# faasm/faabric

Measured on AMD Instinct MI355X. Metric: MPI_Allreduce GB/s + batch-exec msgs/sec, 8-rank world at 1/2/4/8 MI355X, higher is better.
Workload: dtype fp32; 1 GPU; model=faabric composite: 256MB fp32 allreduce + 1MB alltoall + kvtouch batch, global_batch=128, parallelism=mpi1, allreduce_bytes=268435456, pingpong_bytes=0, kv_bytes=4096, full=False, snapshot_bytes_per_rank=0, snapshot_dirty=random-scattered 25pct, random-byte region, gpu=True

## Files before the change

### cpp/bindings/bindings_runtime.cpp

```cpp
#include <pybind11/functional.h>
#include <pybind11/pybind11.h>
#include <pybind11/stl.h>

#include "faabricamd/endpoint.h"
#include "faabricamd/executor.h"
#include "faabricamd/flat.h"
#include "faabricamd/hipipc.h"
#include "faabricamd/mpi.h"
#include "faabricamd/planner.h"
#include "faabricamd/ptp.h"
#include "faabricamd/runner.h"
#include "faabricamd/scheduler.h"
#include "faabricamd/snapshot.h"
#include "faabricamd/state.h"
#include "faabricamd/util.h"
#include "faabricamd/utilextras.h"
#include "faabricamd/dirty.h"
#include <hip/hip_runtime.h>

namespace py = pybind11;
using namespace faabricamd;

namespace faabricamd {
void registerBenchFunctions();
// ... 767 lines not shown
    m.def("prof_summary", &profSummary);
    m.def("prof_clear", &profClear);
    m.def("set_up_crash_handler", &setUpCrashHandler);
    m.def("pin_thread_to_free_cpu", &pinThreadToFreeCpu);

    m.def("_selftest_segfault_tracker", [] {
        py::gil_scoped_release release;
        SegfaultDirtyTracker tracker;
        PageAlignedBuffer buf;
        buf.resize(16 * 4096);
        tracker.startTracking(buf.data(), buf.size());
        buf.data()[3 * 4096 + 5] = 42;
        buf.data()[9 * 4096] = 7;
        tracker.stopTracking(buf.data(), buf.size());
        auto dirty = tracker.getDirtyPages(buf.data(), buf.size());
        int nDirty = 0;
        for (char c : dirty) {
            nDirty += c != 0;
        }
        return nDirty == 2 && dirty[3] == 1 && dirty[9] == 1;
    });

    m.def("_selftest_uffd_tracker", []() -> py::object {
        if (!UffdDirtyTracker::isAvailable()) {
            return py::none();
        }
        bool ok;
        {
            py::gil_scoped_release release;
            UffdDirtyTracker tracker;
            PageAlignedBuffer buf;
            buf.resize(16 * 4096);
            tracker.startTracking(buf.data(), buf.size());
            buf.data()[2 * 4096 + 11] = 42;
            buf.data()[14 * 4096] = 7;
            tracker.stopTracking(buf.data(), buf.size());
            auto dirty = tracker.getDirtyPages(buf.data(), buf.size());
            int nDirty = 0;
            for (char d : dirty) {
                nDirty += d != 0;
            }
            ok = nDirty == 2 && dirty[2] == 1 && dirty[14] == 1;
        }
        return py::bool_(ok);
    });

    m.def("_selftest_softpte_tracker", []() -> py::object {
        if (!SoftPTEDirtyTracker::isAvailable()) {
            return py::none();
        }
        bool ok;
        {
            py::gil_scoped_release release;
            SoftPTEDirtyTracker tracker;
            PageAlignedBuffer buf;
            buf.resize(16 * 4096);
            std::memset(buf.data(), 1, buf.size());
            tracker.startTracking(buf.data(), buf.size());
            buf.data()[5 * 4096 + 3] = 42;
            buf.data()[12 * 4096] = 7;
            tracker.stopTracking(buf.data(), buf.size());
            auto dirty = tracker.getDirtyPages(buf.data(), buf.size());
            ok = dirty.size() == 16 && dirty[5] == 1 && dirty[12] == 1;
        }
        return py::bool_(ok);
    });

    m.def("_debug_runtime_sizes", [] {
        py::dict d;
        d["planner_app_results"] = Planner::get().debugAppResultsCount();
        d["planner_done_apps"] = Planner::get().debugDoneAppsCount();
        d["planner_in_flight"] = Planner::get().debugInFlightCount();
        d["broker_mappings"] = getPointToPointBroker().debugMappingsCount();
        d["broker_channels"] = getPointToPointBroker().debugChannelsCount();
        d["broker_send_seqs"] = getPointToPointBroker().debugSendSeqsCount();
        d["decision_cache"] = DecisionCache::get().size();
        return d;
    });
    m.def("_debug_dispatch_sizes", [] {
        py::dict d;
        d["idle_executors"] = Scheduler::get().debugIdleCount();
        d["planner_msg_index_apps"] = Planner::get().debugMsgIndexCount();
        d["planner_used_slots"] = Planner::get().debugUsedSlots();
        return d;
    });
    m.def("_debug_current_executor_id", [] {
        return ExecutorContext::get().getExecutor()->id;
    });
    m.def("_debug_set_message_result", [](const Message& msg) {
        auto copy = std::make_shared<Message>(msg);
        py::gil_scoped_release release;
        getPlannerClient().setMessageResult(copy);
    });
    m.def("_debug_kv_commit_stats", [] {
        KvCommitStats s = kvCommitStats();
        py::dict d;
        d["launches"] = s.launches;
        d["pages"] = s.pages;
        return d;
    });
    m.def("_debug_kv_sweep_bitmap",
          [](size_t nPages, const std::vector<uint64_t>& setBits) {
              size_t nWords = (nPages + 63) / 64;
              auto words = std::make_unique<std::atomic<uint64_t>[]>(
                std::max<size_t>(nWords, 1));
              for (size_t w = 0; w < nWords; w++) {
                  words[w].store(0);
              }
              for (uint64_t b : setBits) {
                  if (b >= nPages) {
                      throw FaabricException("bit beyond the bitmap");
                  }
                  words[b / 64].fetch_or(1ULL << (b % 64));
              }
              std::vector<uint32_t> pages(nPages);
              size_t n =
                kvSweepDirtyBitmap(words.get(), nPages, pages.data());
              pages.resize(n);
              std::vector<uint64_t> after(nWords);
              for (size_t w = 0; w < nWords; w++) {
                  after[w] = words[w].load();
              }
              return py::make_tuple(pages, after);
          },
          py::arg("n_pages"),
          py::arg("set_bits"));
    m.def("_debug_op_reduce_host",
          [](int op, int dtype, const py::bytes& inBytes,
             const py::bytes& inoutBytes) {
              if (op < 0 || op > (int)MpiOp::PROD || dtype < 0 ||
                  dtype > (int)MpiDataType::BYTE) {
                  throw FaabricException("bad op or dtype");
              }
              std::string in = inBytes;
              std::string inout = inoutBytes;
              size_t elem = mpiTypeSize((MpiDataType)dtype);
              if (in.size() != inout.size() || (in.size() % elem) != 0) {
                  throw FaabricException("operand length mismatch");
              }
              MpiWorld::opReduceHost((MpiOp)op,
                                     (MpiDataType)dtype,
                                     (int)(inout.size() / elem),
                                     (const uint8_t*)in.data(),
                                     (uint8_t*)inout.data());
              return py::bytes(inout.data(), inout.size());
          },
          py::arg("op"),
          py::arg("dtype"),
          py::arg("in_bytes"),
          py::arg("inout_bytes"));
    m.def("wait_batch_done",
          [](int32_t appId, int timeoutMs) {
              py::gil_scoped_release release;
              return getPlannerClient().waitBatchDone(appId, timeoutMs);
          },
          py::arg("app_id"),
          py::arg("timeout_ms") = 30000);
    m.def("set_bound_timeout",
          [](int ms) { getSystemConfig().boundTimeout = ms; });
    m.def("reap_stale_executors", [] {
        py::gil_scoped_release release;
        return Scheduler::get().reapStaleExecutors();
    });
    m.def("register_bench_functions", [] { registerBenchFunctions(); });
    m.def("bench_last_outputs", [] {
        py::dict d;
        for (const auto& [name, data] : benchLastOutputs()) {
            d[py::str(name)] =
// ... 167 lines not shown
```

### cpp/include/faabricamd/executor.h

```cpp
#pragma once

#include <atomic>
#include <functional>
#include <memory>
#include <string>
#include <thread>
#include <vector>

#include "faabricamd/mailbox.h"
#include "faabricamd/messages.h"
#include "faabricamd/queue.h"
#include "faabricamd/dirty.h"
#include "faabricamd/snapshot.h"

namespace faabricamd {

class Executor;


class ExecutorContext
{
  public:
    static bool isSet();
    static void set(Executor* executor,
                    std::shared_ptr<BatchExecuteRequest> req,
                    int msgIdx);
    static void unset();
    static ExecutorContext& get();

    Executor* getExecutor() const { return executor; }
    std::shared_ptr<BatchExecuteRequest> getBatchRequest() const
    {
        return req;
    }
    Message& getMsg();
    int getMsgIdx() const { return msgIdx; }

  private:
    Executor* executor = nullptr;
    std::shared_ptr<BatchExecuteRequest> req;
    int msgIdx = 0;
};


using FaabricFunction = std::function<int32_t(Message&)>;

class FunctionRegistry
{
  public:
    static FunctionRegistry& get();
    void registerFunction(const std::string& user,
                          const std::string& function,
                          FaabricFunction fn);
    FaabricFunction* getFunction(const std::string& user,
                                 const std::string& function);
    void clear();

  private:
    std::mutex mx;
    std::map<std::string, FaabricFunction> functions;
};


struct ExecutorTask
{
    ExecutorTask() = default;
    ExecutorTask(int msgIdxIn, std::shared_ptr<BatchExecuteRequest> reqIn)
      : msgIdx(msgIdxIn)
      , req(std::move(reqIn))
    {}
    int msgIdx = 0;
    std::shared_ptr<BatchExecuteRequest> req;
    bool stop = false;
    bool single = false;
    int64_t enqueueNs = 0;
};

class Executor : public std::enable_shared_from_this<Executor>
{
  public:
    explicit Executor(Message& msg);
    virtual ~Executor();

    void executeTasks(const std::vector<int>& msgIdxs,
                      const std::shared_ptr<BatchExecuteRequest>& req);
    void executeSingleTask(int msgIdx,
                           const std::shared_ptr<BatchExecuteRequest>& req);

    std::vector<std::pair<int32_t, int32_t>> executeThreads(
      std::shared_ptr<BatchExecuteRequest> req,
      const std::vector<SnapshotMergeRegion>& mergeRegions);

    virtual int32_t executeTask(int threadPoolIdx,
                                int msgIdx,
                                std::shared_ptr<BatchExecuteRequest> req);

    virtual std::pair<uint8_t*, size_t> getMemoryView();
    virtual void setMemorySize(size_t newSize);
    void setDeviceMemorySize(size_t newSize);
    std::pair<uint8_t*, size_t> getDeviceMemoryView();
    bool hasDeviceArena() const { return deviceArena != nullptr; }
    virtual void restore(const std::string& snapshotKey);
    virtual void reset(Message& msg);
    virtual void flush();

    bool tryClaim();
    void claim();
    void releaseClaim();
    bool isClaimed() const { return claimed.load(); }
    using IdleExecutors = IdleList<std::shared_ptr<Executor>>;
    void setIdleList(std::shared_ptr<IdleExecutors> list)
    {
        idleList = std::move(list);
    }

    long getMillisSinceLastExec() const;
    void shutdown();

    std::string id;
    Message boundMsg;
    int gpuDevice = -1;

    void setThreadResult(Message& msg,
                         int32_t returnValue,
                         const std::string& key,
                         const std::vector<SnapshotDiffMsg>& diffs);

  protected:
    void threadPoolThread(int poolIdx);
    void handleTaskResult(Message& msg,
                          int32_t returnValue,
                          std::shared_ptr<BatchExecuteRequest> req,
                          bool isLastInBatch);

    int threadPoolSize = 0;
    using TaskMailbox = Mailbox<ExecutorTask>;
    std::vector<std::unique_ptr<TaskMailbox>> threadMailboxes;
    std::vector<std::thread> threadPoolThreads;
    std::unique_ptr<std::atomic<bool>[]> poolThreadUp;
    std::mutex threadsMx;
    void ensurePoolThreadLocked(int poolIdx);
    void postTask(int poolIdx, ExecutorTask&& task);

    std::shared_ptr<IdleExecutors> idleList;

    std::atomic<bool> claimed{ false };
    std::atomic<int64_t> lastExecMs{ 0 };

    std::string lastForkSnapshotKey;
    std::vector<std::string> lastForkRemoteHosts;
    void cleanupForkSnapshot();

    std::shared_ptr<std::atomic<int>> batchCounter;

    PageAlignedBuffer dummyMemory;

    uint8_t* deviceArena = nullptr;
    size_t deviceArenaSize = 0;
};

class ExecutorFactory
{
  public:
    virtual ~ExecutorFactory() = default;
    virtual std::shared_ptr<Executor> createExecutor(Message& msg)
    {
        return std::make_shared<Executor>(msg);
    }
    virtual void flushHost() {}
};

void setExecutorFactory(std::shared_ptr<ExecutorFactory> factory);
std::shared_ptr<ExecutorFactory> getExecutorFactory();

int32_t chainFunction(const std::string& user,
                      const std::string& function,
                      const std::vector<uint8_t>& input);
Message awaitChainedCall(int32_t msgId, int timeoutMs = 60000);

int32_t migrationPoint(const std::vector<uint8_t>& reentryInput);

}
```

### cpp/include/faabricamd/mailbox.h

```cpp
#pragma once

#include <atomic>
#include <climits>
#include <cstddef>
#include <cstdint>
#include <ctime>
#include <mutex>
#include <utility>
#include <vector>

#include <linux/futex.h>
#include <sys/syscall.h>
#include <unistd.h>

namespace faabricamd {

namespace detail {

inline void futexWait(std::atomic<uint32_t>* word,
                      uint32_t expected,
                      int timeoutMs)
{
    static_assert(sizeof(std::atomic<uint32_t>) == sizeof(uint32_t));
    struct timespec ts;
    struct timespec* tsp = nullptr;
    if (timeoutMs > 0) {
        ts.tv_sec = timeoutMs / 1000;
        ts.tv_nsec = (long)(timeoutMs % 1000) * 1000000L;
        tsp = &ts;
    }
    syscall(SYS_futex,
            reinterpret_cast<uint32_t*>(word),
            FUTEX_WAIT_PRIVATE,
            expected,
            tsp,
            nullptr,
            0);
}

inline void futexWake(std::atomic<uint32_t>* word, int n)
{
    syscall(SYS_futex,
            reinterpret_cast<uint32_t*>(word),
            FUTEX_WAKE_PRIVATE,
            n,
            nullptr,
            nullptr,
            0);
}

}

template<typename T, uint32_t SLOTS = 8>
class Mailbox
{
    static_assert(SLOTS >= 2 && (SLOTS & (SLOTS - 1)) == 0,
                  "SLOTS must be a power of two");

  public:
    Mailbox()
    {
        for (uint32_t i = 0; i < SLOTS; i++) {
            slots[i].seq.store(i, std::memory_order_relaxed);
        }
    }
    Mailbox(const Mailbox&) = delete;
    Mailbox& operator=(const Mailbox&) = delete;

    void post(T value)
    {
        uint32_t ticket = tail.fetch_add(1, std::memory_order_relaxed);
        Slot& s = slots[ticket & (SLOTS - 1)];
        uint32_t seen;
        while ((seen = s.seq.load(std::memory_order_acquire)) != ticket) {
            detail::futexWait(&s.seq, seen, 1);
        }
        s.value = std::move(value);
        s.seq.store(ticket + 1, std::memory_order_seq_cst);
        if (sleeping.load(std::memory_order_seq_cst) != 0) {
            detail::futexWake(&s.seq, INT_MAX);
        }
    }

    bool take(T& out, int timeoutMs)
    {
        Slot& s = slots[head & (SLOTS - 1)];
        uint32_t ready = head + 1;
        uint32_t seen = s.seq.load(std::memory_order_acquire);
        if (seen != ready) {
            struct timespec start;
            clock_gettime(CLOCK_MONOTONIC, &start);
            int leftMs = timeoutMs;
            while (true) {
                sleeping.store(1, std::memory_order_seq_cst);
                seen = s.seq.load(std::memory_order_seq_cst);
                if (seen != ready) {
                    detail::futexWait(&s.seq, seen, leftMs);
                    seen = s.seq.load(std::memory_order_acquire);
                }
                sleeping.store(0, std::memory_order_relaxed);
                if (seen == ready) {
                    break;
                }
                if (timeoutMs > 0) {
                    struct timespec now;
                    clock_gettime(CLOCK_MONOTONIC, &now);
                    int64_t goneMs =
                      (int64_t)(now.tv_sec - start.tv_sec) * 1000 +
                      (now.tv_nsec - start.tv_nsec) / 1000000;
                    if (goneMs >= timeoutMs) {
                        return false;
                    }
                    leftMs = (int)(timeoutMs - goneMs);
                }
            }
        }
        out = std::move(s.value);
        s.value = T();
        s.seq.store(head + SLOTS, std::memory_order_release);
        head++;
        return true;
    }

  private:
    struct alignas(64) Slot
    {
        std::atomic<uint32_t> seq{ 0 };
        T value{};
    };
    Slot slots[SLOTS];
    alignas(64) std::atomic<uint32_t> tail{ 0 };
    std::atomic<uint32_t> sleeping{ 0 };
    alignas(64) uint32_t head = 0;
};

template<typename T>
class IdleList
{
  public:
    void push(T value)
    {
        std::lock_guard<std::mutex> lock(mx);
        if (!closed) {
            entries.push_back(std::move(value));
        }
    }

    size_t popMany(size_t n, std::vector<T>& out)
    {
        std::lock_guard<std::mutex> lock(mx);
        size_t got = 0;
        while (got < n && !entries.empty()) {
            out.push_back(std::move(entries.back()));
            entries.pop_back();
            got++;
        }
        return got;
    }

    bool pop(T& out)
    {
        std::lock_guard<std::mutex> lock(mx);
        if (entries.empty()) {
            return false;
        }
        out = std::move(entries.back());
        entries.pop_back();
        return true;
    }

    size_t remove(const T& value)
    {
        std::lock_guard<std::mutex> lock(mx);
        size_t before = entries.size();
        size_t w = 0;
        for (size_t r = 0; r < entries.size(); r++) {
            if (!(entries[r] == value)) {
                if (w != r) {
                    entries[w] = std::move(entries[r]);
                }
                w++;
            }
        }
        entries.resize(w);
        return before - w;
    }

    void close()
    {
        std::vector<T> dropped;
        {
            std::lock_guard<std::mutex> lock(mx);
            closed = true;
            dropped.swap(entries);
        }
    }

    size_t size()
    {
        std::lock_guard<std::mutex> lock(mx);
        return entries.size();
    }

  private:
    std::mutex mx;
    std::vector<T> entries;
    bool closed = false;
};

}
```

### cpp/include/faabricamd/util.h

```cpp
#pragma once

#include <atomic>
#include <cstdarg>
#include <cstdint>
#include <cstring>
#include <string>
#include <vector>

namespace faabricamd {


enum class LogLevel : int
{
    trace = 0,
    debug = 1,
    info = 2,
    warn = 3,
    error = 4,
    off = 5,
};

LogLevel getLogLevel();
void setLogLevel(LogLevel lvl);
void logMessage(LogLevel lvl, const char* fmt, ...)
  __attribute__((format(printf, 2, 3)));

#define FAM_TRACE(...)                                                         \
    ::faabricamd::logMessage(::faabricamd::LogLevel::trace, __VA_ARGS__)
#define FAM_DEBUG(...)                                                         \
    ::faabricamd::logMessage(::faabricamd::LogLevel::debug, __VA_ARGS__)
#define FAM_INFO(...)                                                          \
    ::faabricamd::logMessage(::faabricamd::LogLevel::info, __VA_ARGS__)
#define FAM_WARN(...)                                                          \
    ::faabricamd::logMessage(::faabricamd::LogLevel::warn, __VA_ARGS__)
#define FAM_ERROR(...)                                                         \
    ::faabricamd::logMessage(::faabricamd::LogLevel::error, __VA_ARGS__)


class FaabricException : public std::exception
{
  public:
    explicit FaabricException(std::string msgIn)
      : msg(std::move(msgIn))
    {}
    const char* what() const noexcept override { return msg.c_str(); }

  private:
    std::string msg;
};

class FunctionMigratedException : public FaabricException
{
  public:
    using FaabricException::FaabricException;
};
class FunctionFrozenException : public FaabricException
{
  public:
    using FaabricException::FaabricException;
};

inline constexpr int MIGRATED_FUNCTION_RETURN_VALUE = -99;
inline constexpr int FROZEN_FUNCTION_RETURN_VALUE = -98;


std::string getEnvVar(const std::string& key, const std::string& deflt);
int getEnvVarInt(const std::string& key, int deflt);

int getUsableCores();

struct SystemConfig
{
    std::string logLevel;
    std::string endpointHost;
    std::string plannerHost;
    int plannerPort = 8011;

    std::string batchSchedulerMode;
    int overrideCpuCount = 0;
    int overrideGpuCount = -1;
    int gpuDevice = 0;
    bool gpuDevicePinned = false;
    bool useGpu = true;

    int globalMessageTimeout = 60000;
    int boundTimeout = 30000;

    int functionServerThreads = 4;
    int stateServerThreads = 2;
    int snapshotServerThreads = 2;
    int pointToPointServerThreads = 4;
    int plannerServerThreads = 4;

    std::string dirtyTrackingMode;
    std::string diffingMode;

    std::string stateMode;

    int defaultMpiWorldSize = 5;
    int mpiBasePort = 8020;

    void initialise();
    void print() const;
};

SystemConfig& getSystemConfig();


uint32_t generateGid();
int32_t generateGidInt32();


int64_t getGlobalClockEpochMillis();
int64_t getEpochMicros();
double getSecondsSinceEpoch();


bool startsWith(const std::string& value, const std::string& prefix);
bool endsWith(const std::string& value, const std::string& suffix);
std::string randomString(size_t len);

inline std::vector<uint8_t> stringToBytes(const std::string& s)
{
    return { s.begin(), s.end() };
}
inline std::string bytesToString(const std::vector<uint8_t>& b)
{
    return { b.begin(), b.end() };
}

template<typename T>
void appendBytesOf(std::vector<uint8_t>& out, const T& v)
{
    const auto* p = reinterpret_cast<const uint8_t*>(&v);
    out.insert(out.end(), p, p + sizeof(T));
}

template<typename T>
T readBytesAt(const uint8_t* data, size_t offset)
{
    T v;
    std::memcpy(&v, data + offset, sizeof(T));
    return v;
}


std::string getPrimaryIPForThisHost(const std::string& interface = "");


void setMockMode(bool value);
bool isMockMode();
void setTestMode(bool value);
bool isTestMode();


std::string funcToString(const std::string& user,
                         const std::string& function,
                         int messageId);

std::string getMainThreadSnapshotKey(const std::string& user,
                                     const std::string& function,
                                     int appId);

}
```

### cpp/src/executor.cpp

```cpp
#include "faabricamd/executor.h"
#include "faabricamd/utilextras.h"
#include "faabricamd/mpi.h"
#include "faabricamd/ops.h"
#include "faabricamd/planner.h"

#include <hip/hip_runtime.h>
#include "faabricamd/snapshot.h"
#include "faabricamd/util.h"

#include <algorithm>
#include <cstring>

namespace faabricamd {

void resultBatcherEnqueue(std::shared_ptr<Message> msg);


static thread_local std::shared_ptr<ExecutorContext> currentContext;

bool ExecutorContext::isSet()
{
    return currentContext != nullptr;
}

void ExecutorContext::set(Executor* executor,
                          std::shared_ptr<BatchExecuteRequest> req,
                          int msgIdx)
{
    auto ctx = std::make_shared<ExecutorContext>();
    ctx->executor = executor;
    ctx->req = std::move(req);
    ctx->msgIdx = msgIdx;
    currentContext = ctx;
}

void ExecutorContext::unset()
{
    currentContext = nullptr;
}

ExecutorContext& ExecutorContext::get()
{
    if (!currentContext) {
        throw FaabricException("no executor context set");
    }
    return *currentContext;
}

Message& ExecutorContext::getMsg()
{
    return req->messages.at(msgIdx);
}


FunctionRegistry& FunctionRegistry::get()
{
    static FunctionRegistry reg;
    return reg;
}

void FunctionRegistry::registerFunction(const std::string& user,
                                        const std::string& function,
                                        FaabricFunction fn)
{
    std::lock_guard<std::mutex> lock(mx);
    functions[user + "/" + function] = std::move(fn);
}

FaabricFunction* FunctionRegistry::getFunction(const std::string& user,
                                               const std::string& function)
{
    std::lock_guard<std::mutex> lock(mx);
    auto it = functions.find(user + "/" + function);
    return it == functions.end() ? nullptr : &it->second;
}

void FunctionRegistry::clear()
{
    std::lock_guard<std::mutex> lock(mx);
    functions.clear();
}


Executor::Executor(Message& msg)
  : id(funcToString(msg.user, msg.function, 0) + "_" +
       std::to_string(generateGid()))
  , boundMsg(msg)
{
    threadPoolSize = std::min(getUsableCores(), 64);
    threadMailboxes.resize(threadPoolSize);
    threadPoolThreads.resize(threadPoolSize);
    poolThreadUp = std::make_unique<std::atomic<bool>[]>(threadPoolSize);
    for (int i = 0; i < threadPoolSize; i++) {
        poolThreadUp[i].store(false, std::memory_order_relaxed);
    }
    lastExecMs = getGlobalClockEpochMillis();
}

void Executor::cleanupForkSnapshot()
{
    if (lastForkSnapshotKey.empty()) {
        return;
    }
    DeviceSnapshotRegistry::get().deleteSnapshot(lastForkSnapshotKey);
    SnapshotRegistry::get().deleteSnapshot(lastForkSnapshotKey);
    for (const auto& host : lastForkRemoteHosts) {
        try {
            getSnapshotClient(host)->deleteSnapshot(lastForkSnapshotKey);
        } catch (const std::exception& e) {
            FAM_DEBUG("remote fork-snapshot delete failed: %s", e.what());
        }
    }
    lastForkSnapshotKey.clear();
    lastForkRemoteHosts.clear();
}

Executor::~Executor()
{
    try {
        cleanupForkSnapshot();
    } catch (...) {
    }
    shutdown();
    if (deviceArena != nullptr) {
        hipFree(deviceArena);
    }
}

void Executor::setDeviceMemorySize(size_t newSize)
{
    if (!gpuAvailable()) {
        throw FaabricException("device arena requires a GPU");
    }
    size_t rounded =
      (newSize + DEVICE_PAGE - 1) / DEVICE_PAGE * DEVICE_PAGE;
    if (rounded <= deviceArenaSize) {
        deviceArenaSize = rounded;
        return;
    }
    int dev = gpuDevice >= 0 ? gpuDevice : 0;
    if (hipSetDevice(dev) != hipSuccess) {
        throw FaabricException("hipSetDevice failed");
    }
    uint8_t* fresh = nullptr;
    if (hipMalloc(&fresh, rounded) != hipSuccess) {
        throw FaabricException("device arena alloc failed");
    }
    hipMemset(fresh, 0, rounded);
    if (deviceArena != nullptr) {
        hipMemcpy(fresh, deviceArena, deviceArenaSize,
                  hipMemcpyDeviceToDevice);
        hipFree(deviceArena);
    }
    deviceArena = fresh;
    deviceArenaSize = rounded;
}

std::pair<uint8_t*, size_t> Executor::getDeviceMemoryView()
{
    return { deviceArena, deviceArenaSize };
}

void Executor::shutdown()
{
    std::lock_guard<std::mutex> lock(threadsMx);
    for (int i = 0; i < threadPoolSize; i++) {
        if (threadPoolThreads[i].joinable()) {
            ExecutorTask stopTask;
            stopTask.stop = true;
            threadMailboxes[i]->post(std::move(stopTask));
        }
    }
    for (int i = 0; i < threadPoolSize; i++) {
        if (threadPoolThreads[i].joinable()) {
            threadPoolThreads[i].join();
            poolThreadUp[i].store(false, std::memory_order_release);
        }
    }
}

long Executor::getMillisSinceLastExec() const
{
    return (long)(getGlobalClockEpochMillis() - lastExecMs.load());
}

bool Executor::tryClaim()
{
    bool expected = false;
    return claimed.compare_exchange_strong(expected, true);
}

void Executor::claim()
{
    claimed.store(true);
}

void Executor::releaseClaim()
{
    claimed.store(false);
    if (idleList) {
        idleList->push(shared_from_this());
    }
}

void Executor::ensurePoolThreadLocked(int poolIdx)
{
    if (threadPoolThreads[poolIdx].joinable()) {
        return;
    }
    if (!threadMailboxes[poolIdx]) {
        threadMailboxes[poolIdx] = std::make_unique<TaskMailbox>();
    }
    threadPoolThreads[poolIdx] =
      std::thread([this, poolIdx] { threadPoolThread(poolIdx); });
    poolThreadUp[poolIdx].store(true, std::memory_order_release);
}

void Executor::postTask(int poolIdx, ExecutorTask&& task)
{
    task.enqueueNs = profEnabled() ? profNowNs() : 0;
    threadMailboxes[poolIdx]->post(std::move(task));
}

void Executor::executeSingleTask(
  int msgIdx,
  const std::shared_ptr<BatchExecuteRequest>& req)
{
    if (req->type == BatchExecuteType::THREADS ||
        !req->snapshotKey.empty() ||
        !req->messages.at(msgIdx).snapshotKey.empty() ||
        threadPoolSize == 0) {
        executeTasks({ msgIdx }, req);
        return;
    }
    lastExecMs = getGlobalClockEpochMillis();
    if (!poolThreadUp[0].load(std::memory_order_acquire)) {
        std::lock_guard<std::mutex> lock(threadsMx);
        ensurePoolThreadLocked(0);
    }
    ExecutorTask task(msgIdx, req);
    task.single = true;
    postTask(0, std::move(task));
}

void Executor::executeTasks(const std::vector<int>& msgIdxs,
                            const std::shared_ptr<BatchExecuteRequest>& req)
{
    lastExecMs = getGlobalClockEpochMillis();
    batchCounter = std::make_shared<std::atomic<int>>((int)msgIdxs.size());

    if (!req->snapshotKey.empty()) {
        restore(req->snapshotKey);
    } else if (!req->messages.empty() &&
               !req->messages[msgIdxs[0]].snapshotKey.empty() &&
               req->type != BatchExecuteType::THREADS) {
        const std::string& key = req->messages[msgIdxs[0]].snapshotKey;
        restore(key);
        if (startsWith(key, "migration_")) {
            SnapshotRegistry::get().deleteSnapshot(key);
            DeviceSnapshotRegistry::get().deleteSnapshot(key);
        }
    }

    if (req->type == BatchExecuteType::THREADS &&
        !req->snapshotKey.empty()) {
        auto tracker = getDirtyTracker();
        if (tracker->getType() == "segfault") {
            auto [base, size] = getMemoryView();
            if (size > 0) {
                tracker->startTracking(base, size);
            }
        }
    }

    std::lock_guard<std::mutex> lock(threadsMx);
    for (int msgIdx : msgIdxs) {
        int poolIdx = threadPoolSize == 0 ? 0 : msgIdx % threadPoolSize;
        ensurePoolThreadLocked(poolIdx);
        postTask(poolIdx, ExecutorTask(msgIdx, req));
    }
}

std::vector<std::pair<int32_t, int32_t>> Executor::executeThreads(
  std::shared_ptr<BatchExecuteRequest> req,
  const std::vector<SnapshotMergeRegion>& mergeRegions)
{
    Message& parentMsg = ExecutorContext::get().getMsg();
    std::string key = getMainThreadSnapshotKey(
      parentMsg.user, parentMsg.function, parentMsg.appId);

    bool onDevice = hasDeviceArena();
    {
        Message& pm = ExecutorContext::get().getMsg();
        std::string newKey = getMainThreadSnapshotKey(
          pm.user, pm.function, pm.appId);
        if (!lastForkSnapshotKey.empty() &&
            lastForkSnapshotKey != newKey) {
            cleanupForkSnapshot();
        }
    }
    std::shared_ptr<SnapshotData> snap;
    std::shared_ptr<DeviceSnapshot> dsnap;
    if (onDevice) {
        validateDeviceMergeRegions(mergeRegions, deviceArenaSize);
        auto& dreg = DeviceSnapshotRegistry::get();
        dreg.setMergeRegions(key, mergeRegions);
        if (dreg.snapshotExists(key) &&
            dreg.getSnapshot(key)->size() == deviceArenaSize) {
            dsnap = dreg.getSnapshot(key);
        } else {
            dsnap = std::make_shared<DeviceSnapshot>(
              deviceArenaSize, gpuDevice >= 0 ? gpuDevice : 0);
            dreg.registerSnapshot(key, dsnap);
        }
        dsnap->captureFromDevice(deviceArena);
    } else {
        auto [memBase, memSize] = getMemoryView();
        auto& reg = SnapshotRegistry::get();
        if (reg.snapshotExists(key)) {
            snap = reg.getSnapshot(key);
            snap->copyInData(memBase, memSize, 0);
        } else {
            snap = std::make_shared<SnapshotData>(
              std::vector<uint8_t>(memBase, memBase + memSize));
            reg.registerSnapshot(key, snap);
// ... 97 lines not shown

int32_t Executor::executeTask(int threadPoolIdx,
                              int msgIdx,
                              std::shared_ptr<BatchExecuteRequest> req)
{
    (void)threadPoolIdx;
    Message& msg = req->messages.at(msgIdx);
    FaabricFunction* fn =
      FunctionRegistry::get().getFunction(msg.user, msg.function);
    if (fn == nullptr) {
        throw FaabricException("function not registered: " + msg.user + "/" +
                               msg.function);
    }
    return (*fn)(msg);
}

std::pair<uint8_t*, size_t> Executor::getMemoryView()
{
    return { dummyMemory.data(), dummyMemory.size() };
}

void Executor::setMemorySize(size_t newSize)
{
    dummyMemory.resize(newSize);
}

void Executor::restore(const std::string& snapshotKey)
{
    const auto& conf = getSystemConfig();
    int64_t deadline = getGlobalClockEpochMillis() + conf.boundTimeout;
    while (true) {
        if (DeviceSnapshotRegistry::get().snapshotExists(snapshotKey)) {
            auto dsnap =
              DeviceSnapshotRegistry::get().getSnapshot(snapshotKey);
            if (deviceArenaSize < dsnap->size()) {
                setDeviceMemorySize(dsnap->size());
            }
            hipError_t err = hipMemcpy(deviceArena,
                                       dsnap->data(),
                                       dsnap->size(),
                                       hipMemcpyDeviceToDevice);
            if (err != hipSuccess ||
                hipStreamSynchronize(nullptr) != hipSuccess) {
                throw FaabricException("device snapshot restore failed");
            }
            return;
        }
        if (SnapshotRegistry::get().snapshotExists(snapshotKey)) {
            auto snap = SnapshotRegistry::get().getSnapshot(snapshotKey);
            if (dummyMemory.size() < snap->getSize()) {
                setMemorySize(snap->getSize());
            }
            auto [base, size] = getMemoryView();
            snap->mapToMemory(base, size);
            return;
        }
        if (getGlobalClockEpochMillis() >= deadline) {
            throw FaabricException("snapshot not found: " + snapshotKey);
        }
        usleep(10 * 1000);
    }
}

void Executor::reset(Message& msg)
{
    (void)msg;
}

void Executor::flush()
{
    FunctionRegistry::get().clear();
}

void Executor::setThreadResult(Message& msg,
                               int32_t returnValue,
                               const std::string& key,
                               const std::vector<SnapshotDiffMsg>& diffs)
{
    (void)key;
    (void)diffs;
    msg.returnValue = returnValue;
}

void Executor::threadPoolThread(int poolIdx)
{
    const auto& conf = getSystemConfig();
    TaskMailbox& mailbox = *threadMailboxes[poolIdx];
    while (true) {
        ExecutorTask task;
        if (!mailbox.take(task, conf.boundTimeout)) {
            continue;
        }
        if (task.stop) {
            break;
        }
        if (task.enqueueNs != 0) {
            profRecord("exec_wake",
                       (double)(profNowNs() - task.enqueueNs) / 1e6);
        }

        Message& msg = task.req->messages.at(task.msgIdx);
        int32_t returnValue = 0;
        ExecutorContext::set(this, task.req, task.msgIdx);
        try {
            PROF_START(exec_task)
            returnValue = executeTask(poolIdx, task.msgIdx, task.req);
            PROF_END(exec_task)
            if (msg.isMpi && msg.recordExecGraph &&
                MpiWorldRegistry::get().worldExists(msg.mpiWorldId)) {
                auto counts = MpiWorldRegistry::get()
                                .getWorld(msg.mpiWorldId)
                                .getMsgCountDetails(msg.mpiRank);
                for (const auto& [k, v] : counts) {
                    msg.intExecGraphDetails[k] = v;
                }
            }
        } catch (const FunctionMigratedException&) {
            FAM_DEBUG("task %d migrated", msg.id);
            returnValue = MIGRATED_FUNCTION_RETURN_VALUE;
        } catch (const FunctionFrozenException&) {
            FAM_DEBUG("task %d frozen", msg.id);
            returnValue = FROZEN_FUNCTION_RETURN_VALUE;
        } catch (const std::exception& e) {
            FAM_ERROR("task %d failed: %s", msg.id, e.what());
            returnValue = 1;
            msg.outputData = std::string("Task failed: ") + e.what();
        }
        ExecutorContext::unset();

        bool isLastInBatch =
          task.single || batchCounter->fetch_sub(1) - 1 == 0;
        handleTaskResult(msg, returnValue, task.req, isLastInBatch);
    }
}

void Executor::handleTaskResult(Message& msg,
                                int32_t returnValue,
                                std::shared_ptr<BatchExecuteRequest> req,
                                bool isLastInBatch)
{
    const auto& conf = getSystemConfig();
    msg.returnValue = returnValue;
    msg.executedHost = conf.endpointHost;
    msg.finishTimestamp = getGlobalClockEpochMillis();
    lastExecMs = getGlobalClockEpochMillis();

    bool isThreads = req->type == BatchExecuteType::THREADS;

    if (msg.isMpi && returnValue != MIGRATED_FUNCTION_RETURN_VALUE &&
        returnValue != FROZEN_FUNCTION_RETURN_VALUE &&
        MpiWorldRegistry::get().worldExists(msg.mpiWorldId)) {
        if (MpiWorldRegistry::get()
              .getWorld(msg.mpiWorldId)
              .rankFinished(msg.mpiRank)) {
            MpiWorldRegistry::get().clearWorld(msg.mpiWorldId);
        }
    }

    std::vector<SnapshotDiff> threadDiffs;
    bool deviceThreads =
      isThreads && !req->snapshotKey.empty() &&
      DeviceSnapshotRegistry::get().snapshotExists(req->snapshotKey);
    if (deviceThreads && isLastInBatch) {
        try {
            auto dsnap =
              DeviceSnapshotRegistry::get().getSnapshot(req->snapshotKey);
            auto regions = DeviceSnapshotRegistry::get().getMergeRegions(
              req->snapshotKey);
            uint32_t nd = 0;
            if (!regions.empty()) {
                threadDiffs = dsnap->diffWithRegions(deviceArena, regions);
            } else {
                nd = dsnap->diffXor(deviceArena);
            }
            if (nd > 0) {
                std::vector<uint32_t> pages;
                std::vector<uint8_t> payload;
                dsnap->gatherLastDiffToHost(pages, payload);
                std::vector<uint8_t> packed(4 + pages.size() * 4 +
                                            payload.size());
                uint32_t n = (uint32_t)pages.size();
                std::memcpy(packed.data(), &n, 4);
                std::memcpy(packed.data() + 4,
                            pages.data(),
                            pages.size() * 4);
                std::memcpy(packed.data() + 4 + pages.size() * 4,
                            payload.data(),
                            payload.size());
                threadDiffs.emplace_back(SnapshotDataType::Raw,
                                         SnapshotMergeOperation::XorPages,
                                         0,
                                         packed.data(),
                                         packed.size());
            }
        } catch (const std::exception& e) {
            FAM_ERROR("device thread diff failed: %s", e.what());
        }
    } else if (isThreads && isLastInBatch && !req->snapshotKey.empty()) {
        try {
            auto snap = SnapshotRegistry::get().getSnapshot(req->snapshotKey);
            auto [base, size] = getMemoryView();
            snap->fillGapsWithBytewiseRegions();
            auto tracker = getDirtyTracker();
            if (tracker->getType() == "segfault" && size > 0) {
                tracker->stopTracking(base, size);
                auto dirty = tracker->getDirtyPages(base, size);
                threadDiffs =
                  snap->diffWithDirtyRegions(base, size, dirty);
            } else {
                threadDiffs = snap->diffWithMemory(base, size);
            }
        } catch (const std::exception& e) {
            FAM_ERROR("thread diff failed: %s", e.what());
        }
    }
// ... 172 lines not shown
```

### cpp/src/scheduler.cpp

```cpp
#include "faabricamd/scheduler.h"
#include "faabricamd/utilextras.h"

#include <atomic>
#include <thread>
#include <functional>
#include <condition_variable>
#include "faabricamd/planner.h"
#include "faabricamd/ptp.h"
#include "faabricamd/util.h"
#include "faabricamd/wire.h"

#include <hip/hip_runtime.h>

namespace faabricamd {

static int getNumGpus()
{
    static int n = []() {
        const auto& conf = getSystemConfig();
        if (conf.overrideGpuCount >= 0) {
            return conf.overrideGpuCount;
        }
        if (!conf.useGpu) {
            return 0;
        }
        int count = 0;
        if (hipGetDeviceCount(&count) != hipSuccess) {
            return 0;
        }
        return count;
    }();
    return n;
}

class Scheduler::ReaperThread : public PeriodicBackgroundThread
{
  public:
    void doWork() override { Scheduler::get().reapStaleExecutors(); }
};

Scheduler::Scheduler() = default;

Scheduler& Scheduler::get()
{
    static Scheduler sched;
    return sched;
}

HostResources Scheduler::getThisHostResources()
{
    {
        std::unique_lock<std::shared_mutex> lock(schedMx);
        if (resourcesOverridden) {
            return overriddenResources;
        }
    }
    HostResources res;
    int nGpus = getNumGpus();
    res.slots = nGpus > 0 ? nGpus : getUsableCores();
    res.usedSlots = 0;
    return res;
}

void Scheduler::setThisHostResources(const HostResources& res)
{
    std::unique_lock<std::shared_mutex> lock(schedMx);
    overriddenResources = res;
    resourcesOverridden = true;
}

void Scheduler::executeBatch(std::shared_ptr<BatchExecuteRequest> req)
{
    if (req->messages.empty()) {
        return;
    }
    PROF_START(sched_execute_batch)
    bool isThreads = req->type == BatchExecuteType::THREADS;

    if (isTestMode()) {
        std::unique_lock<std::shared_mutex> lock(schedMx);
        for (const auto& msg : req->messages) {
            recordedMessages.push_back(msg);
        }
    }

    if (isThreads) {
        auto exec = claimExecutor(req->messages[0]);
        std::vector<int> idxs(req->messages.size());
        for (size_t i = 0; i < idxs.size(); i++) {
            idxs[i] = (int)i;
        }
        exec->executeTasks(idxs, req);
    } else {
        size_t n = req->messages.size();
        std::vector<std::shared_ptr<Executor>> execs;
        std::vector<std::string> claimErrors;
        PROF_START(dispatch_claim)
        claimExecutors(*req, execs, claimErrors);
        PROF_END(dispatch_claim)

        PROF_START(dispatch_enqueue)
        for (size_t i = 0; i < n; i++) {
            try {
                if (!execs[i]) {
                    throw FaabricException(claimErrors[i]);
                }
                execs[i]->executeSingleTask((int)i, req);
            } catch (const std::exception& e) {
                FAM_ERROR("claiming executor failed: %s", e.what());
                if (execs[i]) {
                    execs[i]->releaseClaim();
                }
                auto msg = std::make_shared<Message>(req->messages[i]);
                msg->returnValue = 1;
                msg->executedHost = getSystemConfig().endpointHost;
                msg->outputData = std::string("executor claim failed: ") +
                                  e.what();
                getPlannerClient().setMessageResult(msg);
            }
        }
        PROF_END(dispatch_enqueue)
    }
    PROF_END(sched_execute_batch)
}

static std::shared_ptr<Executor> popIdleClaimed(
  Executor::IdleExecutors& idle)
{
    std::shared_ptr<Executor> e;
    while (idle.pop(e)) {
        if (e->tryClaim()) {
            return e;
        }
    }
    return nullptr;
}

std::shared_ptr<Executor> Scheduler::createExecutorLocked(WarmPool& pool,
                                                          Message& msg)
{
    auto exec = getExecutorFactory()->createExecutor(msg);
    exec->claim();
    exec->setIdleList(pool.idle);
    if (getNumGpus() > 0) {
        const auto& conf = getSystemConfig();
        exec->gpuDevice =
          conf.gpuDevicePinned
            ? conf.gpuDevice
            : (int)((pool.list.size()) % (size_t)getNumGpus());
    }
    pool.list.push_back(exec);
    return exec;
}

std::shared_ptr<Executor> Scheduler::claimExecutor(Message& msg)
{
    std::string key = msg.user + "/" + msg.function;

    {
        std::shared_lock<std::shared_mutex> rlock(schedMx);
        auto it = executors.find(key);
        if (it != executors.end()) {
            if (auto e = popIdleClaimed(*it->second->idle)) {
                return e;
            }
        }
    }

    std::unique_lock<std::shared_mutex> lock(schedMx);
    auto& poolPtr = executors[key];
    if (!poolPtr) {
        poolPtr = std::make_unique<WarmPool>();
    }
    if (auto e = popIdleClaimed(*poolPtr->idle)) {
        return e;
    }
    return createExecutorLocked(*poolPtr, msg);
}

void Scheduler::claimExecutors(
  BatchExecuteRequest& req,
  std::vector<std::shared_ptr<Executor>>& execs,
  std::vector<std::string>& errors)
{
    size_t n = req.messages.size();
    execs.assign(n, nullptr);
    errors.assign(n, std::string());

    const Message& first = req.messages[0];
    bool oneFunction = true;
    for (size_t i = 1; i < n && oneFunction; i++) {
        oneFunction = req.messages[i].function == first.function &&
                      req.messages[i].user == first.user;
    }
    if (!oneFunction) {
        for (size_t i = 0; i < n; i++) {
            try {
                execs[i] = claimExecutor(req.messages[i]);
            } catch (const std::exception& e) {
                errors[i] = e.what();
            }
        }
        return;
    }

    std::string key = first.user + "/" + first.function;
    std::vector<std::shared_ptr<Executor>> popped;
    popped.reserve(n);
    size_t got = 0;
    auto takeIdle = [&](Executor::IdleExecutors& idle) {
        while (got < n) {
            popped.clear();
            if (idle.popMany(n - got, popped) == 0) {
                return;
            }
            for (auto& e : popped) {
                if (e->tryClaim()) {
                    execs[got++] = std::move(e);
                }
            }
        }
    };
    {
        std::shared_lock<std::shared_mutex> rlock(schedMx);
        auto it = executors.find(key);
        if (it != executors.end()) {
            takeIdle(*it->second->idle);
        }
    }
    if (got == n) {
        return;
    }

    std::unique_lock<std::shared_mutex> lock(schedMx);
    auto& poolPtr = executors[key];
    if (!poolPtr) {
        poolPtr = std::make_unique<WarmPool>();
    }
    takeIdle(*poolPtr->idle);
    poolPtr->list.reserve(poolPtr->list.size() + (n - got));
    for (; got < n; got++) {
        try {
            execs[got] = createExecutorLocked(*poolPtr, req.messages[got]);
        } catch (const std::exception& e) {
            errors[got] = e.what();
        }
    }
}

int Scheduler::reapStaleExecutors()
{
    std::unique_lock<std::shared_mutex> lock(schedMx);
    const auto& conf = getSystemConfig();
    int reaped = 0;
    for (auto& [key, pool] : executors) {
        auto& list = pool->list;
        for (auto it = list.begin(); it != list.end();) {
            auto& exec = *it;
            if (exec->getMillisSinceLastExec() > conf.boundTimeout &&
                exec->tryClaim()) {
                pool->idle->remove(exec);
                exec->shutdown();
                it = list.erase(it);
                reaped++;
            } else {
                ++it;
            }
        }
    }
    return reaped;
}

void Scheduler::startReaper()
{
    if (!reaper) {
        reaper = std::make_shared<ReaperThread>();
        reaper->startMillis(getSystemConfig().boundTimeout);
    }
}

void Scheduler::stopReaper()
{
    if (reaper) {
        reaper->stop();
        reaper = nullptr;
    }
}

std::shared_ptr<PendingMigration> Scheduler::checkForMigrationOpportunities(
  Message& msg,
  int32_t overwriteNewGroupId)
{
    int32_t newGroupId = 0;
    if (msg.groupIdx == 0 && overwriteNewGroupId == 0) {
        auto req = std::make_shared<BatchExecuteRequest>();
        req->appId = msg.appId;
        req->groupId = msg.groupId;
        req->user = msg.user;
        req->function = msg.function;
        req->type = BatchExecuteType::MIGRATION;
        auto decision = getPlannerClient().callFunctions(req);
        if (decision->appId == DO_NOT_MIGRATE) {
            newGroupId = 0;
        } else if (decision->appId == MUST_FREEZE) {
            newGroupId = MUST_FREEZE;
        } else {
            newGroupId = decision->groupId;
        }
        auto& broker = getPointToPointBroker();
        int32_t payload = newGroupId;
        for (int i = 1; i < msg.groupSize; i++) {
            broker.sendMessage(msg.appId,
                               msg.groupId,
                               PTP_MIGRATION_CHANNEL_OFFSET,
                               i,
                               (const uint8_t*)&payload,
                               sizeof(payload));
        }
    } else if (overwriteNewGroupId != 0) {
        newGroupId = overwriteNewGroupId;
    } else {
        auto data = getPointToPointBroker().recvMessage(
          msg.groupId, PTP_MIGRATION_CHANNEL_OFFSET, msg.groupIdx);
        newGroupId = *(const int32_t*)data.data();
    }

    if (newGroupId == 0) {
        return nullptr;
    }

    auto migration = std::make_shared<PendingMigration>();
    migration->appId = msg.appId;
    migration->groupIdx = msg.groupIdx;
    migration->srcHost = getSystemConfig().endpointHost;

    if (newGroupId == MUST_FREEZE) {
        migration->appId = MUST_FREEZE;
        return migration;
    }

    migration->groupId = newGroupId;
    auto decision = getPlannerClient().getSchedulingDecision(msg.appId);
    for (int i = 0; i < decision.nFunctions; i++) {
// ... 259 lines not shown
```

### cpp/src/util.cpp

```cpp
#include "faabricamd/util.h"

#include <arpa/inet.h>
#include <chrono>
#include <cstdio>
#include <cstdlib>
#include <ifaddrs.h>
#include <mutex>
#include <net/if.h>
#include <random>
#include <sys/types.h>
#include <thread>
#include <unistd.h>

namespace faabricamd {


static std::atomic<int> logLevelValue{ -1 };

static LogLevel parseLogLevel(const std::string& s)
{
    if (s == "trace") {
        return LogLevel::trace;
    }
    if (s == "debug") {
// ... 31 lines not shown

void logMessage(LogLevel lvl, const char* fmt, ...)
{
    if ((int)lvl < (int)getLogLevel()) {
        return;
    }
    static const char* names[] = { "TRACE", "DEBUG", "INFO",
                                   "WARN",  "ERROR", "OFF" };
    char body[2048];
    va_list args;
    va_start(args, fmt);
    vsnprintf(body, sizeof(body), fmt, args);
    va_end(args);

    auto now = std::chrono::system_clock::now();
    auto ms = std::chrono::duration_cast<std::chrono::milliseconds>(
                now.time_since_epoch())
                .count();
    time_t secs = (time_t)(ms / 1000);
    struct tm tmv;
    localtime_r(&secs, &tmv);
    char ts[32];
    strftime(ts, sizeof(ts), "%H:%M:%S", &tmv);

    fprintf(stderr,
            "[%s.%03d] [%lu] [%s] %s\n",
            ts,
            (int)(ms % 1000),
            (unsigned long)(std::hash<std::thread::id>{}(
                              std::this_thread::get_id()) %
                            100000),
            names[(int)lvl],
            body);
}


std::string getEnvVar(const std::string& key, const std::string& deflt)
{
    const char* v = ::getenv(key.c_str());
    if (v == nullptr || *v == '\0') {
        return deflt;
    }
    return std::string(v);
}

int getEnvVarInt(const std::string& key, int deflt)
{
    const char* v = ::getenv(key.c_str());
    if (v == nullptr || *v == '\0') {
        return deflt;
    }
    return atoi(v);
}

int getUsableCores()
{
    int override = getEnvVarInt("OVERRIDE_CPU_COUNT", 0);
    if (override > 0) {
        return override;
    }
    unsigned int n = std::thread::hardware_concurrency();
    return n == 0 ? 1 : (int)n;
}

void SystemConfig::initialise()
{
    logLevel = getEnvVar("LOG_LEVEL", "info");
    endpointHost = getEnvVar("ENDPOINT_HOST", "");
    if (endpointHost.empty()) {
        endpointHost = getPrimaryIPForThisHost();
    }
    plannerHost = getEnvVar("PLANNER_HOST", "localhost");
    plannerPort = getEnvVarInt("PLANNER_PORT", 8011);

    batchSchedulerMode = getEnvVar("BATCH_SCHEDULER_MODE", "bin-pack");
    overrideCpuCount = getEnvVarInt("OVERRIDE_CPU_COUNT", 0);
    overrideGpuCount = getEnvVarInt("OVERRIDE_GPU_COUNT", -1);
    gpuDevice = getEnvVarInt("FAABRIC_GPU_DEVICE", 0);
    gpuDevicePinned = !getEnvVar("FAABRIC_GPU_DEVICE", "").empty();
    useGpu = getEnvVarInt("FAABRIC_USE_GPU", 1) != 0;

    globalMessageTimeout = getEnvVarInt("GLOBAL_MESSAGE_TIMEOUT", 60000);
    boundTimeout = getEnvVarInt("BOUND_TIMEOUT", 30000);

    functionServerThreads = getEnvVarInt("FUNCTION_SERVER_THREADS", 4);
    stateServerThreads = getEnvVarInt("STATE_SERVER_THREADS", 2);
    snapshotServerThreads = getEnvVarInt("SNAPSHOT_SERVER_THREADS", 2);
    pointToPointServerThreads = getEnvVarInt("POINT_TO_POINT_SERVER_THREADS", 4);
    plannerServerThreads = getEnvVarInt("PLANNER_SERVER_THREADS", 4);

    dirtyTrackingMode = getEnvVar("DIRTY_TRACKING_MODE", "compare");
    diffingMode = getEnvVar("DIFFING_MODE", "xor");

    stateMode = getEnvVar("STATE_MODE", "inmemory");

    defaultMpiWorldSize = getEnvVarInt("DEFAULT_MPI_WORLD_SIZE", 5);
    mpiBasePort = getEnvVarInt("MPI_BASE_PORT", 8020);
}

void SystemConfig::print() const
{
    FAM_INFO("--- faabric-mi355x config ---");
    FAM_INFO("endpointHost       %s", endpointHost.c_str());
    FAM_INFO("plannerHost        %s:%d", plannerHost.c_str(), plannerPort);
    FAM_INFO("batchScheduler     %s", batchSchedulerMode.c_str());
    FAM_INFO("dirtyTrackingMode  %s", dirtyTrackingMode.c_str());
    FAM_INFO("diffingMode        %s", diffingMode.c_str());
}

SystemConfig& getSystemConfig()
{
    static SystemConfig conf;
    static std::once_flag flag;
    std::call_once(flag, [&]() { conf.initialise(); });
    return conf;
}


static std::atomic<uint64_t> gidCounter{ 0 };

static uint64_t gidKey()
{
    static uint64_t key = []() {
        std::random_device rd;
        std::mt19937_64 gen(rd() ^ (uint64_t)::getpid());
        return gen();
    }();
    return key;
}

uint32_t generateGid()
{
    uint64_t c = gidCounter.fetch_add(1, std::memory_order_relaxed);
    uint32_t r = (uint32_t)((gidKey() + c) % (uint64_t)INT32_MAX);
    return r == 0 ? 1 : r;
}

int32_t generateGidInt32()
{
    return (int32_t)generateGid();
}


int64_t getGlobalClockEpochMillis()
{
    return std::chrono::duration_cast<std::chrono::milliseconds>(
             std::chrono::system_clock::now().time_since_epoch())
      .count();
}

int64_t getEpochMicros()
{
    return std::chrono::duration_cast<std::chrono::microseconds>(
             std::chrono::system_clock::now().time_since_epoch())
      .count();
}

double getSecondsSinceEpoch()
{
    return (double)getEpochMicros() / 1e6;
}


bool startsWith(const std::string& value, const std::string& prefix)
{
    return value.rfind(prefix, 0) == 0;
// ... 99 lines not shown
```

Baseline: 240,100 msgs/sec.

## Dispatch large batches via carrier executors draining a shared work queue

```diff
diff --git a/cpp/bindings/bindings_runtime.cpp b/cpp/bindings/bindings_runtime.cpp
--- a/cpp/bindings/bindings_runtime.cpp
+++ b/cpp/bindings/bindings_runtime.cpp
@@ -873,8 +873,18 @@
         d["idle_executors"] = Scheduler::get().debugIdleCount();
         d["planner_msg_index_apps"] = Planner::get().debugMsgIndexCount();
         d["planner_used_slots"] = Planner::get().debugUsedSlots();
+        DrainStats& ds = drainStats();
+        d["drain_batches"] = ds.batches.load();
+        d["drain_tasks_by_carrier"] = ds.tasksByCarrier.load();
+        d["drain_tasks_by_owner"] = ds.tasksByOwner.load();
+        d["drain_stall_fallbacks"] = ds.stallFallbacks.load();
         return d;
     });
+    m.def("set_dispatch_carriers", [](int n) {
+        getSystemConfig().dispatchCarriers = n < 0 ? 0 : n;
+    });
+    m.def("get_dispatch_carriers",
+          [] { return getSystemConfig().dispatchCarriers; });
     m.def("_debug_current_executor_id", [] {
         return ExecutorContext::get().getExecutor()->id;
     });
diff --git a/cpp/include/faabricamd/executor.h b/cpp/include/faabricamd/executor.h
--- a/cpp/include/faabricamd/executor.h
+++ b/cpp/include/faabricamd/executor.h
@@ -61,6 +61,18 @@
     std::map<std::string, FaabricFunction> functions;
 };
 
+
+struct DrainEntry;
+using BatchDrain = DrainQueue<DrainEntry>;
+
+struct DrainStats
+{
+    std::atomic<uint64_t> batches{ 0 };
+    std::atomic<uint64_t> tasksByCarrier{ 0 };
+    std::atomic<uint64_t> tasksByOwner{ 0 };
+    std::atomic<uint64_t> stallFallbacks{ 0 };
+};
+DrainStats& drainStats();
 
 struct ExecutorTask
 {
@@ -74,6 +86,13 @@
     bool stop = false;
     bool single = false;
     int64_t enqueueNs = 0;
+    std::shared_ptr<BatchDrain> drain;
+};
+
+struct DrainEntry
+{
+    std::shared_ptr<Executor> exec;
+    ExecutorTask task;
 };
 
 class Executor : public std::enable_shared_from_this<Executor>
@@ -85,7 +104,16 @@
     void executeTasks(const std::vector<int>& msgIdxs,
                       const std::shared_ptr<BatchExecuteRequest>& req);
     void executeSingleTask(int msgIdx,
-                           const std::shared_ptr<BatchExecuteRequest>& req);
+                           const std::shared_ptr<BatchExecuteRequest>& req,
+                           std::shared_ptr<BatchDrain> drain = nullptr);
+
+    void runTask(ExecutorTask& task, int poolIdx = 0);
+
+    static void carryDrain(BatchDrain& drain);
+    bool isCarrying() const
+    {
+        return carryingMask.load(std::memory_order_acquire) != 0;
+    }
 
     std::vector<std::pair<int32_t, int32_t>> executeThreads(
       std::shared_ptr<BatchExecuteRequest> req,
@@ -145,6 +173,7 @@
     std::shared_ptr<IdleExecutors> idleList;
 
     std::atomic<bool> claimed{ false };
+    std::atomic<uint32_t> carryingMask{ 0 };
     std::atomic<int64_t> lastExecMs{ 0 };
 
     std::string lastForkSnapshotKey;
diff --git a/cpp/include/faabricamd/mailbox.h b/cpp/include/faabricamd/mailbox.h
--- a/cpp/include/faabricamd/mailbox.h
+++ b/cpp/include/faabricamd/mailbox.h
@@ -5,6 +5,7 @@
 #include <cstddef>
 #include <cstdint>
 #include <ctime>
+#include <memory>
 #include <mutex>
 #include <utility>
 #include <vector>
@@ -34,6 +35,22 @@
             FUTEX_WAIT_PRIVATE,
             expected,
             tsp,
+            nullptr,
+            0);
+}
+
+inline void futexWaitUs(std::atomic<uint32_t>* word,
+                        uint32_t expected,
+                        int timeoutUs)
+{
+    struct timespec ts;
+    ts.tv_sec = timeoutUs / 1000000;
+    ts.tv_nsec = (long)(timeoutUs % 1000000) * 1000L;
+    syscall(SYS_futex,
+            reinterpret_cast<uint32_t*>(word),
+            FUTEX_WAIT_PRIVATE,
+            expected,
+            &ts,
             nullptr,
             0);
 }
@@ -135,6 +152,75 @@
 };
 
 template<typename T>
+class DrainQueue
+{
+  public:
+    explicit DrainQueue(size_t n)
+      : entries(n)
+      , flags(new std::atomic<uint8_t>[n])
+    {
+        for (size_t i = 0; i < n; i++) {
+            flags[i].store(0, std::memory_order_relaxed);
+        }
+    }
+    DrainQueue(const DrainQueue&) = delete;
+    DrainQueue& operator=(const DrainQueue&) = delete;
+
+    size_t size() const { return entries.size(); }
+    T& entry(size_t i) { return entries[i]; }
+
+    void startAt(size_t i) { cursor.store(i, std::memory_order_relaxed); }
+
+    bool takeNext(size_t& idx)
+    {
+        size_t n = entries.size();
+        while (cursor.load(std::memory_order_relaxed) < n) {
+            size_t i = cursor.fetch_add(1, std::memory_order_relaxed);
+            if (i >= n) {
+                break;
+            }
+            if (takeAt(i)) {
+                idx = i;
+                return true;
+            }
+        }
+        return false;
+    }
+
+    bool takeAt(size_t i)
+    {
+        if (flags[i].exchange(1, std::memory_order_acq_rel) != 0) {
+            return false;
+        }
+        uint32_t now = count.fetch_add(1, std::memory_order_acq_rel) + 1;
+        if (now == entries.size()) {
+            done.store(1, std::memory_order_seq_cst);
+            detail::futexWake(&done, INT_MAX);
+        }
+        return true;
+    }
+
+    uint32_t takenCount() const
+    {
+        return count.load(std::memory_order_acquire);
+    }
+
+    void waitAllTaken(int timeoutUs)
+    {
+        if (done.load(std::memory_order_seq_cst) == 0) {
+            detail::futexWaitUs(&done, 0, timeoutUs);
+        }
+    }
+
+  private:
+    std::vector<T> entries;
+    std::unique_ptr<std::atomic<uint8_t>[]> flags;
+    alignas(64) std::atomic<size_t> cursor{ 0 };
+    alignas(64) std::atomic<uint32_t> count{ 0 };
+    std::atomic<uint32_t> done{ 0 };
+};
+
+template<typename T>
 class IdleList
 {
   public:
diff --git a/cpp/include/faabricamd/util.h b/cpp/include/faabricamd/util.h
--- a/cpp/include/faabricamd/util.h
+++ b/cpp/include/faabricamd/util.h
@@ -86,6 +86,8 @@
     int globalMessageTimeout = 60000;
     int boundTimeout = 30000;
 
+    int dispatchCarriers = 8;
+
     int functionServerThreads = 4;
     int stateServerThreads = 2;
     int snapshotServerThreads = 2;
diff --git a/cpp/src/executor.cpp b/cpp/src/executor.cpp
--- a/cpp/src/executor.cpp
+++ b/cpp/src/executor.cpp
@@ -82,12 +82,18 @@
 }
 
 
+DrainStats& drainStats()
+{
+    static DrainStats stats;
+    return stats;
+}
+
 Executor::Executor(Message& msg)
   : id(funcToString(msg.user, msg.function, 0) + "_" +
        std::to_string(generateGid()))
   , boundMsg(msg)
 {
-    threadPoolSize = std::min(getUsableCores(), 64);
+    threadPoolSize = std::max(2, std::min(getUsableCores(), 64));
     threadMailboxes.resize(threadPoolSize);
     threadPoolThreads.resize(threadPoolSize);
     poolThreadUp = std::make_unique<std::atomic<bool>[]>(threadPoolSize);
@@ -224,7 +230,8 @@
 
 void Executor::executeSingleTask(
   int msgIdx,
-  const std::shared_ptr<BatchExecuteRequest>& req)
+  const std::shared_ptr<BatchExecuteRequest>& req,
+  std::shared_ptr<BatchDrain> drain)
 {
     if (req->type == BatchExecuteType::THREADS ||
         !req->snapshotKey.empty() ||
@@ -234,13 +241,20 @@
         return;
     }
     lastExecMs = getGlobalClockEpochMillis();
-    if (!poolThreadUp[0].load(std::memory_order_acquire)) {
+    int poolIdx = 0;
+    uint32_t busy = carryingMask.load(std::memory_order_acquire);
+    if (busy != 0) {
+        int firstFree = __builtin_ctz(~busy);
+        poolIdx = firstFree < threadPoolSize ? firstFree : 0;
+    }
+    if (!poolThreadUp[poolIdx].load(std::memory_order_acquire)) {
         std::lock_guard<std::mutex> lock(threadsMx);
-        ensurePoolThreadLocked(0);
+        ensurePoolThreadLocked(poolIdx);
     }
     ExecutorTask task(msgIdx, req);
     task.single = true;
-    postTask(0, std::move(task));
+    task.drain = std::move(drain);
+    postTask(poolIdx, std::move(task));
 }
 
 void Executor::executeTasks(const std::vector<int>& msgIdxs,
@@ -504,10 +518,61 @@
     msg.returnValue = returnValue;
 }
 
+void Executor::runTask(ExecutorTask& task, int poolIdx)
+{
+    if (deviceArena != nullptr && gpuDevice >= 0) {
+        (void)hipSetDevice(gpuDevice);
+    }
+
+    Message& msg = task.req->messages.at(task.msgIdx);
+    int32_t returnValue = 0;
+    ExecutorContext::set(this, task.req, task.msgIdx);
+    try {
+        PROF_START(exec_task)
+        returnValue = executeTask(poolIdx, task.msgIdx, task.req);
+        PROF_END(exec_task)
+        if (msg.isMpi && msg.recordExecGraph &&
+            MpiWorldRegistry::get().worldExists(msg.mpiWorldId)) {
+            auto counts = MpiWorldRegistry::get()
+                            .getWorld(msg.mpiWorldId)
+                            .getMsgCountDetails(msg.mpiRank);
+            for (const auto& [k, v] : counts) {
+                msg.intExecGraphDetails[k] = v;
+            }
+        }
+    } catch (const FunctionMigratedException&) {
+        FAM_DEBUG("task %d migrated", msg.id);
+        returnValue = MIGRATED_FUNCTION_RETURN_VALUE;
+    } catch (const FunctionFrozenException&) {
+        FAM_DEBUG("task %d frozen", msg.id);
+        returnValue = FROZEN_FUNCTION_RETURN_VALUE;
+    } catch (const std::exception& e) {
+        FAM_ERROR("task %d failed: %s", msg.id, e.what());
+        returnValue = 1;
+        msg.outputData = std::string("Task failed: ") + e.what();
+    }
+    ExecutorContext::unset();
+
+    bool isLastInBatch =
+      task.single || batchCounter->fetch_sub(1) - 1 == 0;
+    handleTaskResult(msg, returnValue, task.req, isLastInBatch);
+}
+
+void Executor::carryDrain(BatchDrain& drain)
+{
+    size_t idx;
+    while (drain.takeNext(idx)) {
+        DrainEntry entry = std::move(drain.entry(idx));
+        drainStats().tasksByCarrier.fetch_add(1, std::memory_order_relaxed);
+        entry.exec->runTask(entry.task);
+    }
+}
+
 void Executor::threadPoolThread(int poolIdx)
 {
     const auto& conf = getSystemConfig();
     TaskMailbox& mailbox = *threadMailboxes[poolIdx];
+    const uint32_t carryBit = poolIdx < 32 ? (1u << poolIdx) : 0;
     while (true) {
         ExecutorTask task;
         if (!mailbox.take(task, conf.boundTimeout)) {
@@ -520,39 +585,14 @@
             profRecord("exec_wake",
                        (double)(profNowNs() - task.enqueueNs) / 1e6);
         }
-
-        Message& msg = task.req->messages.at(task.msgIdx);
-        int32_t returnValue = 0;
-        ExecutorContext::set(this, task.req, task.msgIdx);
-        try {
-            PROF_START(exec_task)
-            returnValue = executeTask(poolIdx, task.msgIdx, task.req);
-            PROF_END(exec_task)
-            if (msg.isMpi && msg.recordExecGraph &&
-                MpiWorldRegistry::get().worldExists(msg.mpiWorldId)) {
-                auto counts = MpiWorldRegistry::get()
-                                .getWorld(msg.mpiWorldId)
-                                .getMsgCountDetails(msg.mpiRank);
-                for (const auto& [k, v] : counts) {
-                    msg.intExecGraphDetails[k] = v;
-                }
-            }
-        } catch (const FunctionMigratedException&) {
-            FAM_DEBUG("task %d migrated", msg.id);
-            returnValue = MIGRATED_FUNCTION_RETURN_VALUE;
-        } catch (const FunctionFrozenException&) {
-            FAM_DEBUG("task %d frozen", msg.id);
-            returnValue = FROZEN_FUNCTION_RETURN_VALUE;
-        } catch (const std::exception& e) {
-            FAM_ERROR("task %d failed: %s", msg.id, e.what());
-            returnValue = 1;
-            msg.outputData = std::string("Task failed: ") + e.what();
-        }
-        ExecutorContext::unset();
-
-        bool isLastInBatch =
-          task.single || batchCounter->fetch_sub(1) - 1 == 0;
-        handleTaskResult(msg, returnValue, task.req, isLastInBatch);
+        if (!task.drain) {
+            runTask(task, poolIdx);
+            continue;
+        }
+        carryingMask.fetch_or(carryBit, std::memory_order_acq_rel);
+        runTask(task, poolIdx);
+        carryDrain(*task.drain);
+        carryingMask.fetch_and(~carryBit, std::memory_order_acq_rel);
     }
 }
 
diff --git a/cpp/src/scheduler.cpp b/cpp/src/scheduler.cpp
--- a/cpp/src/scheduler.cpp
+++ b/cpp/src/scheduler.cpp
@@ -33,6 +33,11 @@
     return n;
 }
 
+static constexpr size_t DRAIN_MIN_BATCH_PER_CARRIER = 4;
+
+static constexpr int DRAIN_STALL_INTERVAL_US = 200;
+static constexpr uint32_t DRAIN_MIN_ADVANCE = 50;
+
 class Scheduler::ReaperThread : public PeriodicBackgroundThread
 {
   public:
@@ -99,17 +104,19 @@
         claimExecutors(*req, execs, claimErrors);
         PROF_END(dispatch_claim)
 
-        PROF_START(dispatch_enqueue)
-        for (size_t i = 0; i < n; i++) {
+        auto handOff = [&req](size_t i,
+                              const std::shared_ptr<Executor>& exec,
+                              const std::string& claimError,
+                              std::shared_ptr<BatchDrain> drain) {
             try {
-                if (!execs[i]) {
-                    throw FaabricException(claimErrors[i]);
+                if (!exec) {
+                    throw FaabricException(claimError);
                 }
-                execs[i]->executeSingleTask((int)i, req);
+                exec->executeSingleTask((int)i, req, std::move(drain));
             } catch (const std::exception& e) {
                 FAM_ERROR("claiming executor failed: %s", e.what());
-                if (execs[i]) {
-                    execs[i]->releaseClaim();
+                if (exec) {
+                    exec->releaseClaim();
                 }
                 auto msg = std::make_shared<Message>(req->messages[i]);
                 msg->returnValue = 1;
@@ -117,6 +124,68 @@
                 msg->outputData = std::string("executor claim failed: ") +
                                   e.what();
                 getPlannerClient().setMessageResult(msg);
+            }
+        };
+
+        size_t carriers = (size_t)getSystemConfig().dispatchCarriers;
+        bool drained = carriers > 0 &&
+                       n >= carriers * DRAIN_MIN_BATCH_PER_CARRIER &&
+                       req->type == BatchExecuteType::FUNCTIONS &&
+                       req->snapshotKey.empty();
+        for (size_t i = 0; drained && i < n; i++) {
+            const Message& m = req->messages[i];
+            drained = execs[i] != nullptr && !m.isMpi &&
+                      m.snapshotKey.empty();
+        }
+
+        PROF_START(dispatch_enqueue)
+        if (!drained) {
+            for (size_t i = 0; i < n; i++) {
+                handOff(i, execs[i], claimErrors[i], nullptr);
+            }
+        } else {
+            auto drain = std::make_shared<BatchDrain>(n);
+            for (size_t i = 0; i < carriers; i++) {
+                drain->takeAt(i);
+            }
+            drain->startAt(carriers);
+            for (size_t i = carriers; i < n; i++) {
+                DrainEntry& e = drain->entry(i);
+                e.exec = std::move(execs[i]);
+                e.task.msgIdx = (int)i;
+                e.task.req = req;
+                e.task.single = true;
+            }
+            auto& stats = drainStats();
+            stats.batches.fetch_add(1, std::memory_order_relaxed);
+            stats.tasksByOwner.fetch_add(carriers,
+                                         std::memory_order_relaxed);
+            for (size_t i = 0; i < carriers; i++) {
+                handOff(i, execs[i], claimErrors[i], drain);
+            }
+
+            uint32_t seen = drain->takenCount();
+            while (seen < n) {
+                drain->waitAllTaken(DRAIN_STALL_INTERVAL_US);
+                uint32_t now = drain->takenCount();
+                if (now >= n) {
+                    break;
+                }
+                if (now - seen >= DRAIN_MIN_ADVANCE) {
+                    seen = now;
+                    continue;
+                }
+                stats.stallFallbacks.fetch_add(1,
+                                               std::memory_order_relaxed);
+                for (size_t i = carriers; i < n; i++) {
+                    if (drain->takeAt(i)) {
+                        DrainEntry e = std::move(drain->entry(i));
+                        stats.tasksByOwner.fetch_add(
+                          1, std::memory_order_relaxed);
+                        handOff(i, e.exec, std::string(), nullptr);
+                    }
+                }
+                break;
             }
         }
         PROF_END(dispatch_enqueue)
@@ -258,7 +327,7 @@
         for (auto it = list.begin(); it != list.end();) {
             auto& exec = *it;
             if (exec->getMillisSinceLastExec() > conf.boundTimeout &&
-                exec->tryClaim()) {
+                !exec->isCarrying() && exec->tryClaim()) {
                 pool->idle->remove(exec);
                 exec->shutdown();
                 it = list.erase(it);
diff --git a/cpp/src/util.cpp b/cpp/src/util.cpp
--- a/cpp/src/util.cpp
+++ b/cpp/src/util.cpp
@@ -137,6 +137,10 @@
 
     globalMessageTimeout = getEnvVarInt("GLOBAL_MESSAGE_TIMEOUT", 60000);
     boundTimeout = getEnvVarInt("BOUND_TIMEOUT", 30000);
+    dispatchCarriers = getEnvVarInt("FAABRIC_DISPATCH_CARRIERS", 8);
+    if (dispatchCarriers < 0) {
+        dispatchCarriers = 0;
+    }
 
     functionServerThreads = getEnvVarInt("FUNCTION_SERVER_THREADS", 4);
     stateServerThreads = getEnvVarInt("STATE_SERVER_THREADS", 2);
```

Measured after the change: 217,600 msgs/sec. 0.906x the previous value.
